# uiuc-iml/RA-SLAM

Hardware: AMD Instinct MI355X
Metric: depth+semantic frames/sec integrated @640x480, 5mm voxels (higher is better)
Workload: dtype f32

## Files before the change

ra-slam_amd/csrc/kernels_cand.h:

```cpp
#pragma once
#include "kernels_alloc.h"

namespace ratsdf {

constexpr int kCandSegs = 64;
constexpr int kCandCountStride = 32;
constexpr uint32_t kCandReserve = 32;
constexpr unsigned long long kCandEmpty = ~0ull;


struct CandJob {
  FrameParams P;
  const float* depth;
  const uint8_t* rgb;
  const float* ht;
  const float* lt;
  float4* texA;
  uint32_t* texB;
  CandSet set;
  uint32_t first_tile, n_tiles;
  uint32_t tiles_per_wg;
  uint32_t tiles_x;
  uint32_t tiles_x_magic;
};
inline uint32_t cand_tiles_magic(uint32_t tiles_x) { return tiles_x > 1 ? 0xFFFFFFFFu / tiles_x + 1u : 0u; }

constexpr uint32_t kCandLdsSlots = 512;

struct CandLds {
  unsigned long long keys[kCandLdsSlots];
  uint32_t ranks[kCandLdsSlots];
  uint32_t n, base;
};

__device__ inline void cand_append(const CandSet& cs, uint32_t seg, uint32_t k0, uint32_t k1,
                                   uint32_t rank, Ctl* ctl) {
  const uint32_t pos = atomicAdd(&cs.count[seg * kCandCountStride], 1u);
  if (pos < cs.seg_cap) {
    cs.list[(size_t)seg * cs.seg_cap + pos] = make_uint4(k0, k1, rank, 0u);
  } else {
    set_error(ctl, RATSDF_ERR_CAPACITY);
  }
}

__device__ inline bool cand_lds_insert(CandLds& L, unsigned long long key, uint32_t h, uint32_t rank) {
  uint32_t s = h & (kCandLdsSlots - 1);
  for (uint32_t guard = 0; guard < 32; ++guard) {
    unsigned long long k = L.keys[s];
    if (k == kCandEmpty) k = atomicCAS(&L.keys[s], kCandEmpty, key);
    if (k == kCandEmpty || k == key) {
      atomicMin(&L.ranks[s], rank);
      return true;
    }
    s = (s + 1) & (kCandLdsSlots - 1);
  }
  return false;
}

template <typename Overflow>
__device__ inline void cand_pixel_work(const CandJob& J, CandLds& L, uint32_t wg, Ctl* ctl, uint32_t reserved_at,
                                       Overflow overflow) {
  const FrameParams& P = J.P;
  const uint32_t wave = (uint32_t)__builtin_amdgcn_readfirstlane((int)(threadIdx.x >> 6));
  const int lane = threadIdx.x & 63;
  if (J.tiles_per_wg == 4 && (wg | 15u) < (J.n_tiles + 3) / 4) wg = (wg & ~15u) | ((wg & 7u) << 1) | ((wg >> 3) & 1u);
  const uint32_t rel = wg * J.tiles_per_wg + wave;
  const uint32_t tile = J.first_tile + rel;
  const uint32_t sup = tile >> 2, sub = tile & 3u;
  const uint32_t srow = J.tiles_x > 1 ? __umulhi(sup, J.tiles_x_magic) : sup;
  const uint32_t scol = sup - srow * J.tiles_x;
  const int px = (int)scol * 16 + (lane & 15);
  const int py = (int)srow * 16 + (int)sub * 4 + (lane >> 4);
  const bool inb = wave < J.tiles_per_wg && rel < J.n_tiles && px < P.W && py < P.H;
  const int pix = inb ? py * P.W + px : 0;
  float d = 0.f, hv = 1.f, lv = 1.f;
  uint32_t c0 = 0, c1 = 0, c2 = 0;
#ifdef RATSDF_STAMPS
  unsigned long long pt[5];
  pt[0] = clock64();
#endif
  if (inb) {
    c0 = J.rgb[3 * pix];
    c1 = J.rgb[3 * pix + 1];
    c2 = J.rgb[3 * pix + 2];
    d = J.depth[pix];
    if (P.has_sem) {
      hv = J.ht[pix];
      lv = J.lt[pix];
    }
  }
  const uint32_t c = c0 | (c1 << 8) | (c2 << 16);

  if (threadIdx.x == 0) L.base = reserved_at;
  const V3 pimg{(float)px, (float)py, 1.f};
  const V3 pc = intr_mul(P.Ki, pimg);
  const float r = sqrtf(pc.x * pc.x + (pc.y * pc.y + pc.z * pc.z));
  if (inb) {
    float ln = 0.f;
    if (P.has_sem) ln = __logf(hv) - __logf(lv);
    const Recip rmd = make_recip(P.md);
    const float wn = (1 - (recip_safe(P.md) ? div_shared(d, rmd) : d / P.md)) * 4;
    J.texA[pix] = make_float4(d, r, ln, wn);
    J.texB[pix] = c;
  }
  bool valid = inb && !(d == 0 || d > P.md);
  if (RATSDF_DBG(P, 1)) return;
#ifdef RATSDF_STAMPS
  pt[1] = clock64();
#endif

  const V3 pcd{pc.x * d, pc.y * d, pc.z * d};
  const V3 pw = se3_apply(P.Ti, pcd);
  if (P.shard_count > 1) {
    const float lo = (pw.x - P.trunc) / P.vs - 2.5f, hi = (pw.x + P.trunc) / P.vs + 2.5f;
    if (lo > -32000.f && hi < 32000.f) {
      const int s_lo = ((int)floorf(lo) >> 3) >> P.shard_slab_bits, s_hi = ((int)floorf(hi) >> 3) >> P.shard_slab_bits;
      const uint32_t u = (uint32_t)(s_lo + P.shard_bias);
      const uint32_t m_lo = u - __umulhi(u, P.shard_magic) * (uint32_t)P.shard_count;
      uint32_t k0 = (uint32_t)P.shard_rank + (uint32_t)P.shard_count - m_lo;
      if (k0 >= (uint32_t)P.shard_count) k0 -= (uint32_t)P.shard_count;
      if (k0 > (uint32_t)(s_hi - s_lo)) valid = false;
    }
    if (!__any(valid)) return;
  }
  const Recip rr = make_recip(r), rvs = make_recip(P.vs);
  const bool vs_ok = recip_safe(P.vs);
  const V3 dc{div_shared(pc.x, rr), div_shared(pc.y, rr), div_shared(pc.z, rr)};
  const V3 dw = quat_rotate(P.Ti.q, dc);
  const V3 sw{pw.x - dw.x * P.trunc, pw.y - dw.y * P.trunc, pw.z - dw.z * P.trunc};
  V3 dg, sg;
  if (vs_ok && __all(fabsf(sw.x) < 1e18f && fabsf(sw.y) < 1e18f && fabsf(sw.z) < 1e18f)) {
    dg = V3{div_shared(dw.x, rvs), div_shared(dw.y, rvs), div_shared(dw.z, rvs)};
    sg = V3{div_shared(sw.x, rvs), div_shared(sw.y, rvs), div_shared(sw.z, rvs)};
  } else {
    dg = V3{dw.x / P.vs, dw.y / P.vs, dw.z / P.vs};
    sg = V3{sw.x / P.vs, sw.y / P.vs, sw.z / P.vs};
  }
  const float two_tr = 2 * P.trunc;
  const V3 rg{two_tr * dg.x, two_tr * dg.y, two_tr * dg.z};
  int steps = f2i(ceilf(fmaxf(fmaxf(fabsf(rg.x), fabsf(rg.y)), fabsf(rg.z)) / RATSDF_BLOCK_LEN));
// ... 34 lines not shown
    const uint32_t k0 = act ? key0(bx, by) : kInf;
    const uint32_t k1 = act ? key1(bz) : kInf;
    const uint32_t n0 = (uint32_t)__builtin_amdgcn_update_dpp(0, (int)k0, 0x138, 0xF, 0xF, false);
    const uint32_t n1 = (uint32_t)__builtin_amdgcn_update_dpp(0, (int)k1, 0x138, 0xF, 0xF, false);
    const bool dup = (k0 == prev0 && k1 == prev1) || (lane > 0 && k0 == n0 && k1 == n1);
    if (act && !dup && shard_owned(bx, P) && !RATSDF_DBG(P, 2)) {
      const uint32_t rank = (uint32_t)pix * (uint32_t)P.S + (uint32_t)i;
      const unsigned long long key = (unsigned long long)k0 | ((unsigned long long)k1 << 32);
      if (!cand_lds_insert(L, key, (uint32_t)(bx + by * 17 + bz * 41), rank)) overflow(bx, by, bz, k0, k1, rank);
    }
    if (act) {
      prev0 = k0;
      prev1 = k1;
    }
    p.x += st.x;
    p.y += st.y;
    p.z += st.z;
#ifdef RATSDF_STAMPS
    pt[4] += 1;
#endif
  }
#ifdef RATSDF_STAMPS
  pt[3] = clock64();
  if (threadIdx.x == 0 && (wg & 15) == 0) {
    atomicAdd(&ctl->tstamps[11], pt[1] - pt[0]);
    atomicAdd(&ctl->tstamps[12], pt[2] - pt[1]);
    atomicAdd(&ctl->tstamps[13], pt[3] - pt[2]);
    atomicAdd(&ctl->tstamps[14], pt[4]);
    atomicAdd(&ctl->tstamps[15], 1ull);
  }
#endif
}

__device__ inline void cand_pixels_role(const CandJob& J, uint32_t wg, Ctl* ctl, CandLds& L) {
  const uint32_t nthreads = block_threads();
  for (uint32_t i = threadIdx.x; i < kCandLdsSlots; i += nthreads) {
    L.keys[i] = kCandEmpty;
    L.ranks[i] = kInf;
  }
  const uint32_t seg = (J.first_tile + wg) & (kCandSegs - 1);
  const uint32_t reserve = kCandReserve * ((J.tiles_per_wg + 3) / 4);
  uint32_t reserved_at = 0;
  if (threadIdx.x == 0) {
    L.n = 0;
    uint32_t opaque_zero;
    asm("v_mov_b32 %0, 0" : "=v"(opaque_zero));
    reserved_at = atomicAdd(&J.set.count[seg * kCandCountStride + opaque_zero], reserve);
  }
#ifdef RATSDF_STAMPS
  unsigned long long cs[4];
  cs[0] = clock64();
  unsigned long long* ws = (ctl->debug_buf && RATSDF_DBG(J.P, 8))
                               ? ctl->debug_buf + (size_t)(((J.first_tile / 4 + wg) * 4 + (threadIdx.x >> 6)) & 16383) * 8
                               : nullptr;
  if (ws && (threadIdx.x & 63) == 0) { ws[0] = cs[0]; ws[5] = wall_clock64(); }
#endif
  asm volatile("s_waitcnt lgkmcnt(0)\n\ts_barrier" ::: "memory");
#ifdef RATSDF_STAMPS
  cs[1] = clock64();
#endif
  if ((threadIdx.x >> 6) < J.tiles_per_wg)
    cand_pixel_work(J, L, wg, ctl, reserved_at, [&](int, int, int, uint32_t k0, uint32_t k1, uint32_t rank) {
      cand_append(J.set, (J.first_tile + wg) & (kCandSegs - 1), k0, k1, rank, ctl);
    });
#ifdef RATSDF_STAMPS
  cs[2] = clock64();
#endif
  asm volatile("s_waitcnt lgkmcnt(0)\n\ts_barrier" ::: "memory");
#ifdef RATSDF_STAMPS
  cs[3] = clock64();
  if (threadIdx.x == 0 && (wg & 15) == 0) {
    atomicAdd(&ctl->stamps[14], cs[1] - cs[0]);
    atomicAdd(&ctl->stamps[15], cs[2] - cs[1]);
    atomicAdd(&ctl->stamps[16], cs[3] - cs[2]);
    atomicAdd(&ctl->stamps[17], 1ull);
  }
#endif
  constexpr uint32_t kMaxPerThread = kCandLdsSlots / 64;
  uint32_t pos[kMaxPerThread];
#pragma unroll
  for (uint32_t k = 0; k < kMaxPerThread; ++k) {
    pos[k] = kInf;
    if (k * nthreads < kCandLdsSlots) {
      const uint32_t i = threadIdx.x + k * nthreads;
      if (i < kCandLdsSlots && L.keys[i] != kCandEmpty) pos[k] = atomicAdd(&L.n, 1u);
    }
  }
  asm volatile("s_waitcnt lgkmcnt(0)\n\ts_barrier" ::: "memory");
  const uint32_t n = L.n;
  const uint32_t base = L.base;
  uint32_t base2 = 0;
  if (n > reserve) {
    __syncthreads();
    if (threadIdx.x == 0) L.base = atomicAdd(&J.set.count[seg * kCandCountStride], n - reserve);
    __syncthreads();
    base2 = L.base;
  }
  if (base + reserve > J.set.seg_cap || (n > reserve && base2 + (n - reserve) > J.set.seg_cap)) {
    if (threadIdx.x == 0) set_error(ctl, RATSDF_ERR_CAPACITY);
    return;
  }
  uint4* out = J.set.list + (size_t)seg * J.set.seg_cap;
#pragma unroll
  for (uint32_t k = 0; k < kMaxPerThread; ++k) {
    const uint32_t i = threadIdx.x + k * nthreads;
    if (pos[k] != kInf) {
      const unsigned long long key = L.keys[i];
      const uint32_t at = pos[k] < reserve ? base + pos[k] : base2 + (pos[k] - reserve);
      out[at] = make_uint4((uint32_t)key, (uint32_t)(key >> 32), L.ranks[i], 0u);
    }
  }
  for (uint32_t i = n + threadIdx.x; i < reserve; i += nthreads)
    out[base + i] = make_uint4(kInf, kInf, kInf, 0u);
#ifdef RATSDF_STAMPS
  if (threadIdx.x == 0 && (wg & 15) == 0) atomicAdd(&ctl->stamps[18], (unsigned long long)clock64() - cs[3]);
  if (ws && (threadIdx.x & 63) == 0) {
    ws[1] = cs[1]; ws[2] = cs[2]; ws[3] = cs[3]; ws[4] = clock64(); ws[6] = wall_clock64();
  }
#endif
}

__device__ inline bool wave_block_visible_full(bool want, int bx, int by, int bz,
                                               const FrameParams& P) {
  const int lane = threadIdx.x & 63;
  unsigned long long todo = __ballot(want);
  unsigned long long ok = 0;
  while (todo) {
    unsigned long long packed = 0;
#pragma unroll
    for (int k = 0; k < 8; ++k) {
      unsigned long long o = 0xFFull;
      if (todo) {
        o = (unsigned long long)(__ffsll((long long)todo) - 1);
        todo &= todo - 1;
      }
      packed |= o << (8 * k);
    }
    const uint32_t own = (uint32_t)(packed >> (8 * (lane >> 3))) & 0xFFu;
    const int src = own == 0xFFu ? 0 : (int)own;
    const int cbx = __shfl(bx, src), cby = __shfl(by, src), cbz = __shfl(bz, src);
    const int c = lane & 7;
    const int cx = (int16_t)((int16_t)(cbx << 3) + ((c >> 0) & 1) * 7);
    const int cy = (int16_t)((int16_t)(cby << 3) + ((c >> 1) & 1) * 7);
    const int cz = (int16_t)((int16_t)(cbz << 3) + ((c >> 2) & 1) * 7);
    const bool v = own == 0xFFu || voxel_visible(cx, cy, cz, P);
    const unsigned long long b = __ballot(v);
#pragma unroll
    for (int k = 0; k < 8; ++k) {
      const unsigned long long o = (packed >> (8 * k)) & 0xFFull;
      if (o != 0xFFull && ((b >> (8 * k)) & 0xFFull) == 0xFFull) ok |= 1ull << o;
    }
  }
// ... 97 lines not shown
```

ra-slam_amd/csrc/kernels_frame.h:

```cpp
#pragma once
#include "kernels_integrate.h"

namespace ratsdf {

struct FrameJob {
  FrameParams P;
  const float* depth;
  const uint8_t* rgb;
  const float* ht;
  const float* lt;
  uint32_t par;
  uint32_t pad;
};
typedef const FrameJob __attribute__((address_space(4))) * JobPtr;

struct AheadGeom {
  uint32_t first_tile, n_tiles, tiles_per_wg, tiles_x, tiles_x_magic;
};

__device__ inline CandJob make_cand_job(EnginePtr E, JobPtr J, const AheadGeom& g) {
  CandJob j;
  j.P = ld_const(&J->P);
  j.depth = J->depth;
  j.rgb = J->rgb;
  j.ht = J->ht;
  j.lt = J->lt;
  const uint32_t par = J->par;
  j.texA = E->texA[par];
  j.texB = E->texB[par];
  j.set = ld_const(&E->cand[par]);
  j.first_tile = g.first_tile;
  j.n_tiles = g.n_tiles;
  j.tiles_per_wg = g.tiles_per_wg;
  j.tiles_x = g.tiles_x;
  j.tiles_x_magic = g.tiles_x_magic;
  return j;
}

constexpr uint32_t kFrontLdsWords = 2 * kSmallCarve + 16;
constexpr uint32_t kTailPerThread = 8;
constexpr uint32_t kTailReqMax = kTailPerThread * 256;
constexpr uint32_t kTailWinMax = kFreshCap;
constexpr uint32_t kTailBins = 512;
constexpr uint32_t kTailLdsWords = 32 + 5 * kTailWinMax;
static_assert(kTailBins <= kTailWinMax && kTailBins == 2 * 256, "two bins per thread; the cursors' memory is reused");

__device__ inline bool front_arrive(FrameCtl* F, uint32_t wg, uint32_t n_wg, Ctl* ctl) {
  __shared__ uint32_t arrived_last;
#ifdef RATSDF_STAMPS
  __shared__ unsigned long long arrive_t[3];
  if (threadIdx.x == 0) arrive_t[0] = wall_clock64();
#endif
  asm volatile("s_waitcnt vmcnt(0)" ::: "memory");
  __syncthreads();
#ifdef RATSDF_STAMPS
  if (threadIdx.x == 0) arrive_t[1] = wall_clock64();
#endif
  if (threadIdx.x == 0) {
    const uint32_t sub = wg % kArriveSubs;
    const uint32_t members = (n_wg - sub + kArriveSubs - 1) / kArriveSubs;
    uint32_t last = 0;
    if (__hip_atomic_fetch_add(&F->arrive[sub * kListStride], 1u, __ATOMIC_RELAXED, __HIP_MEMORY_SCOPE_AGENT) ==
        members - 1u) {
      const uint32_t tops = n_wg < kArriveSubs ? n_wg : kArriveSubs;
      last = __hip_atomic_fetch_add(&F->arrive_top, 1u, __ATOMIC_RELAXED, __HIP_MEMORY_SCOPE_AGENT) == tops - 1u;
    }
    arrived_last = last;
#ifdef RATSDF_STAMPS
// ... 212 lines not shown
    F->alloc_base = (uint32_t)nf;
    F->n_win = take;
    F->n_winlist = total;
    F->pending = 1;
    F->front_done = 1;
    ctl->num_free = nf - (int32_t)take;
    atomicMin(&ctl->free_low, nf - (int32_t)take);
    atomicAdd(&ctl->paths[0], 1ull);
#ifdef RATSDF_STAMPS
    tt[3] = wall_clock64();
    const unsigned long long T0 = __hip_atomic_load(&ctl->tstamps[0], __ATOMIC_RELAXED, __HIP_MEMORY_SCOPE_AGENT);
    for (int i = 0; i < 4; ++i) ctl->tstamps[4 + i] += tt[i] - T0;
    ctl->tstamps[8] += 1;
    ctl->tstamps[9] += n;
    ctl->tstamps[10] += total;
#endif
  }
}

template <bool kTail, typename Ahead>
__device__ inline void front_body(const Table& tab, const FrameParams& P, uint32_t n_vis_wg,
                                  const CandSet& cand, uint32_t cand_parts, Request* req,
                                  uint32_t req_cap, SlowRequest* slow, uint32_t slow_cap, VisItem* vis,
                                  uint32_t seg_cap, const Pool& pool, const CarveBufs& cb, Ctl* ctl,
                                  uint32_t par, ratsdf_frame_stats* stats, uint32_t tail, Ahead ahead,
                                  uint32_t* role_lds) {
  static_assert(sizeof(CandLds) <= kFrontLdsWords * 4 && kVisListCap <= 2 * kSmallCarve &&
                    sizeof(ReqBuf) <= kFrontLdsWords * 4,
                "role LDS");
  const uint32_t n_cons_wg = kCandSegs * cand_parts;
  const uint32_t n_dir_wg = n_vis_wg + n_cons_wg + kReleaseWGs;
  if (blockIdx.x >= n_dir_wg) {
    const CandJob job = ahead();
    cand_pixels_role(job, blockIdx.x - n_dir_wg, ctl, *reinterpret_cast<CandLds*>(role_lds));
    return;
  }
  FrameCtl* F = &ctl->fr[par];
  FrameCtl* Fp = &ctl->fr[par ^ 1u];
  if (kTail && (tail & 2u)) __builtin_amdgcn_s_setprio(3);
#ifdef RATSDF_STAMPS
  if (blockIdx.x == 0 && threadIdx.x == 0)
    __hip_atomic_store(&ctl->tstamps[0], (unsigned long long)wall_clock64(), __ATOMIC_RELAXED, __HIP_MEMORY_SCOPE_AGENT);
#endif
  bool expired = false;
  auto gate = [&]() {
    const GateResult g = carve_resolve_gate(tab, cb, ctl, Fp, RATSDF_DBG(P, 20));
    expired = expired || g == kGateExpired;
    return g;
  };
  if (blockIdx.x >= n_vis_wg + n_cons_wg) {
    if (!RATSDF_DBG(P, 12) && gate() != kGateExpired)
      carve_release_role(tab, pool, cb, ctl, Fp, blockIdx.x - n_vis_wg - n_cons_wg, role_lds);
  } else if (blockIdx.x >= n_vis_wg) {
    if (!RATSDF_DBG(P, 11)) {
      const uint32_t c = blockIdx.x - n_vis_wg;
      cand_consume_role(tab, P, cand, c % kCandSegs, c / kCandSegs, cand_parts, req, req_cap, slow,
                        slow_cap, ctl, F, gate, *reinterpret_cast<ReqBuf*>(role_lds));
    }
  } else {
    if (!RATSDF_DBG(P, 3)) visible_append_role(tab, P, blockIdx.x, n_vis_wg, vis, seg_cap, ctl, F, gate, role_lds);
  }
  if constexpr (kTail) {
    if ((tail & 1u) && !expired && front_arrive(F, blockIdx.x, n_dir_wg, ctl))
      front_tail_role(tab, P, cand, req, req_cap, vis, seg_cap, pool, cb, ctl, par, stats, role_lds);
  }
}

template <bool kTail>
__global__ __launch_bounds__(256) __attribute__((amdgpu_num_sgpr(80), amdgpu_waves_per_eu(8))) void k_front(
    Table tab, FrameParams P, uint32_t n_vis_wg, CandSet cand, uint32_t cand_parts, Request* req,
    uint32_t req_cap,
    SlowRequest* slow, uint32_t slow_cap, VisItem* vis, uint32_t seg_cap, Pool pool, CarveBufs cb,
    Ctl* ctl, uint32_t par, ratsdf_frame_stats* stats, uint32_t tail, CandJob ahead) {
  __shared__ __attribute__((aligned(16))) uint32_t role_lds[kFrontLdsWords];
  front_body<kTail>(tab, P, n_vis_wg, cand, cand_parts, req, req_cap, slow, slow_cap, vis, seg_cap, pool, cb,
                    ctl, par, stats, tail, [&]() { return ahead; }, role_lds);
}

__global__ __launch_bounds__(256) __attribute__((amdgpu_num_sgpr(80), amdgpu_waves_per_eu(8))) void k_front_inline(
    Table tab, uint32_t n_vis_wg, uint32_t n_now_wg, Request* req, uint32_t req_cap, SlowRequest* slow,
    uint32_t slow_cap, VisItem* vis, uint32_t seg_cap, Pool pool, CarveBufs cb, Ctl* ctl, uint32_t par, CandJob now,
    CandJob ahead) {
  static_assert((kInlineReqOffsetWords * 4u + sizeof(ReqBuf)) <= kFrontLdsWords * 4u, "role LDS");
  __shared__ __attribute__((aligned(16))) uint32_t role_lds[kFrontLdsWords];
  const uint32_t n_dir_wg = n_vis_wg + n_now_wg + kReleaseWGs;
  if (blockIdx.x >= n_dir_wg) {
    cand_pixels_role(ahead, blockIdx.x - n_dir_wg, ctl, *reinterpret_cast<CandLds*>(role_lds));
    return;
  }
  FrameCtl* F = &ctl->fr[par];
  FrameCtl* Fp = &ctl->fr[par ^ 1u];
  auto gate = [&]() { return carve_resolve_gate(tab, cb, ctl, Fp, RATSDF_DBG(now.P, 20)); };
  if (blockIdx.x >= n_vis_wg + n_now_wg) {
    if (gate() != kGateExpired)
      carve_release_role(tab, pool, cb, ctl, Fp, blockIdx.x - n_vis_wg - n_now_wg, role_lds);
  } else if (blockIdx.x >= n_vis_wg) {
    cand_inline_role(now, blockIdx.x - n_vis_wg, tab, req, req_cap, slow, slow_cap, ctl, F, gate, role_lds);
  } else {
    visible_append_role(tab, now.P, blockIdx.x, n_vis_wg, vis, seg_cap, ctl, F, gate, role_lds);
  }
}

template <bool kTail>
__global__ __launch_bounds__(256) __attribute__((amdgpu_num_sgpr(80), amdgpu_waves_per_eu(8))) void k_front_g(
    EnginePtr engs, JobPtr cur, JobPtr nxt, uint32_t n_vis_wg, uint32_t cand_parts, uint32_t tail, AheadGeom ag) {
  __shared__ __attribute__((aligned(16))) uint32_t role_lds[kFrontLdsWords];
  EnginePtr E = engs + blockIdx.y;
  JobPtr J = cur + blockIdx.y;
  const uint32_t par = J->par;
  const RankBufs rb = ld_const(&E->rb);
  front_body<kTail>(ld_const(&E->tab), ld_const(&J->P), n_vis_wg, ld_const(&E->cand[par]), cand_parts, rb.req,
             rb.req_cap, E->slow, E->slow_cap, E->vis, E->seg_cap, ld_const(&E->pool),
             ld_const(&E->cb[par ^ 1u]), E->ctl, par, E->stats, tail,
             [&]() { return make_cand_job(E, nxt + blockIdx.y, ag); }, role_lds);
}

__device__ inline void serial_frame_role(const Table& tab, const Pool& pool, const RankBufs& rb,
                                         const CarveBufs& cb, Ctl* ctl, uint32_t par,
                                         ratsdf_frame_stats* stats, unsigned long long* skeys) {
#ifdef RATSDF_STAMPS
// ... 162 lines not shown
  cand_pixels_role(job, blockIdx.x, E->ctl, L);
}

template <int VPL, bool kTail>
__global__ __launch_bounds__(VPL == 1 ? 512 : RATSDF_INTEG_NT) __attribute__((amdgpu_num_sgpr(80), amdgpu_waves_per_eu(VPL <= 2 ? 8 : (VPL == 4 ? 5 : 3)))) void k_integrate_g(
    EnginePtr engs, JobPtr cur, JobPtr nxt, uint32_t n_int_wg, uint32_t n_serial_wg, uint32_t n_ahead_wg,
    uint32_t commit_rot, AheadGeom ag) {
  constexpr bool tail_on = kTail;
  __shared__ __attribute__((aligned(16))) uint32_t role_lds[kIntegLdsWords];
  EnginePtr E = engs + blockIdx.y;
  JobPtr J = cur + blockIdx.y;
  const uint32_t par = J->par;
  if (__builtin_expect(blockIdx.x >= n_serial_wg + n_ahead_wg, 1)) {
    const uint32_t ibid = blockIdx.x - n_serial_wg - n_ahead_wg;
    const bool fused = n_serial_wg != 0;
    IntegArgs A;
    A.rgbw = E->pool.rgbw;
    A.tsdf = E->pool.tsdf;
    A.segm = E->pool.segm;
    A.texA = E->texA[par];
    A.texB = E->texB[par];
    A.vis = E->vis;
    A.seg_cap = E->seg_cap;
    A.F = &E->ctl->fr[par];
    A.upd_wg = E->cb[par].upd_wg;
    A.par = par;
    const FrameParams P = ld_const(&J->P);
#include "integrate_body.inc"
    return;
  }
  if (blockIdx.x >= n_serial_wg) {
    if (VPL != 1) {
      const CandJob ahead = make_cand_job(E, nxt + blockIdx.y, ag);
      cand_pixels_role(ahead, blockIdx.x - n_serial_wg, E->ctl, *reinterpret_cast<CandLds*>(role_lds));
    }
    return;
  }
  if (blockIdx.x == 0) {
    const uint32_t nwords = ((uint32_t)(J->P.W * J->P.H) * (uint32_t)J->P.S + 31u) / 32u;
    serial_workgroup(E, par, nwords, role_lds, RATSDF_DBG(J->P, 21));
  } else {
    serial_helper(E, par, role_lds, blockIdx.x, RATSDF_DBG(J->P, 22));
  }
}

}
```

ra-slam_amd/csrc/kernels_integrate.h:

```cpp
#pragma once
#include "kernels_carve.h"

namespace ratsdf {

template <typename Op>
__device__ inline uint32_t wave_reduce_dpp(uint32_t v, uint32_t identity, Op op) {
  v = op(v, (uint32_t)__builtin_amdgcn_update_dpp((int)identity, (int)v, 0xB1, 0xF, 0xF, false));
  v = op(v, (uint32_t)__builtin_amdgcn_update_dpp((int)identity, (int)v, 0x4E, 0xF, 0xF, false));
  v = op(v, (uint32_t)__builtin_amdgcn_update_dpp((int)identity, (int)v, 0x141, 0xF, 0xF, false));
  v = op(v, (uint32_t)__builtin_amdgcn_update_dpp((int)identity, (int)v, 0x140, 0xF, 0xF, false));
  v = op(v, (uint32_t)__builtin_amdgcn_update_dpp((int)identity, (int)v, 0x142, 0xA, 0xF, false));
  v = op(v, (uint32_t)__builtin_amdgcn_update_dpp((int)identity, (int)v, 0x143, 0xC, 0xF, false));
  return (uint32_t)__builtin_amdgcn_readlane((int)v, 63);
}
__device__ inline uint32_t wave_sum(uint32_t v) {
  return wave_reduce_dpp(v, 0u, [](uint32_t a, uint32_t b) { return a + b; });
}

template <int N>
struct VecIO;
template <>
struct VecIO<8> {
  static __device__ inline void load(const uint32_t* p, uint32_t (&v)[8]) {
    const uint4 a = reinterpret_cast<const uint4*>(p)[0], b = reinterpret_cast<const uint4*>(p)[1];
// ... 688 lines not shown
  }
}

#ifndef RATSDF_INTEG_NT
#define RATSDF_INTEG_NT 256
#endif

struct IntegArgs {
  uint32_t* rgbw;
  float* tsdf;
  float* segm;
  const float4* texA;
  const uint32_t* texB;
  const VisItem* vis;
  uint32_t seg_cap;
  FrameCtl* F;
  uint32_t* upd_wg;
  uint32_t par;
};

template <int VPL, bool kTail>
__global__ __launch_bounds__(VPL == 1 ? 512 : RATSDF_INTEG_NT) __attribute__((amdgpu_num_sgpr(80), amdgpu_waves_per_eu(VPL <= 2 ? 8 : (VPL == 4 ? 5 : 3)))) void k_integrate(
    IntegArgs A, FrameParams P, EnginePtr E, uint32_t n_int_wg, uint32_t n_serial_wg, uint32_t n_ahead_wg,
    uint32_t commit_rot, CandJob ahead) {
  constexpr bool tail_on = kTail;
  __shared__ __attribute__((aligned(16))) uint32_t role_lds[kIntegLdsWords];
  if (__builtin_expect(blockIdx.x >= n_serial_wg + n_ahead_wg, 1)) {
    const uint32_t ibid = blockIdx.x - n_serial_wg - n_ahead_wg;
    const bool fused = n_serial_wg != 0;
#include "integrate_body.inc"
    return;
  }
  if (blockIdx.x >= n_serial_wg) {
    if (VPL != 1) cand_pixels_role(ahead, blockIdx.x - n_serial_wg, E->ctl, *reinterpret_cast<CandLds*>(role_lds));
    return;
  }
  if (blockIdx.x == 0)
    serial_workgroup(E, A.par, ((uint32_t)(P.W * P.H) * (uint32_t)P.S + 31u) / 32u, role_lds, RATSDF_DBG(P, 21));
  else
    serial_helper(E, A.par, role_lds, blockIdx.x, RATSDF_DBG(P, 22));
}

}
```

ra-slam_amd/csrc/ratsdf_engine.hip:

```cpp
#include <hip/hip_runtime.h>
#include <hip/hip_ext.h>

#include <cmath>
#include <cstdio>
#include <cstdlib>
#include <cstring>
#include <new>
#include <algorithm>
#include <atomic>
#include <condition_variable>
#include <mutex>
#include <thread>
#include <vector>

#include "kernels_frame.h"
#include "kernels_mesh.h"
#include "kernels_sample.h"
#include "kernels_esdf.h"
#include "kernels_fuse.h"
#include "hip_mem.h"
#include "../../include/ratsdf_sample.h"
#include "../../include/ratsdf_esdf.h"

static_assert(sizeof(ratsdf_sample) == 32 && offsetof(ratsdf_sample, flags) == 25, "ratsdf_sample layout");
// ... 384 lines not shown
  int ensure_stage(size_t npix);
  EngineDev record() const;
  int upload_record();
  RankBufs rank_bufs(uint32_t nranks) const;
  int alloc_rank(uint32_t nranks, unsigned par, const CandJob* next = nullptr, bool frame = false);
  int commit_pass(uint32_t nranks, unsigned par);
  int settle();
  void abandon_pipeline(int frames_launched = 0, bool clear_next = false);
  CarveBufs carve_bufs(unsigned par) const;
  int select(int mode, const GridBounds& gb, uint32_t* count_slot);
  struct FrameIn {
    const void *rgb, *depth, *ht, *lt;
    const ratsdf_intrinsics* K;
    const ratsdf_pose* T;
    static FrameIn of(const void* rgb, const void* depth, const void* ht, const void* lt, const ratsdf_intrinsics* K,
                      const ratsdf_pose* T) {
      if (!ht || !lt) ht = lt = nullptr;
      return FrameIn{rgb, depth, ht, lt, K, T};
    }
    static FrameIn at(size_t i, const void* const* rgb, const void* const* depth, const void* const* ht,
                      const void* const* lt, const ratsdf_intrinsics* K, const ratsdf_pose* T) {
      return of(rgb[i], depth[i], ht ? ht[i] : nullptr, lt ? lt[i] : nullptr, &K[i], &T[i]);
    }
  };
  FrameParams frame_params(const FrameIn& in, int H, int W, float md) const;
  void fill_job(FrameJob& j, const FrameIn& in, int H, int W, float md, unsigned par) const;
  CandJob cand_job(const FrameIn& in, const FrameParams& P, unsigned par) const;
  int frame(const FrameIn& cur, const FrameIn* next, int H, int W, float md);
  int sticky();
  int read_small(void* dst, const void* dev_src, size_t bytes);
  FrameParams base_params() const;
  struct Geom {
    unsigned n_vis_wg, parts, n_front_wg, n_cand_wg, grid;
    AheadGeom a, b, c;
  };
  Geom geometry(int H, int W, bool has_next, int split_a, int split_b) const;
  int lookahead_split(size_t npix) const;
  bool graph_eligible(int n, int H, int W) const;
  struct StageSlot {
    uint8_t *h, *d;
    size_t npix;
    FrameIn input(const ratsdf_intrinsics* K, const ratsdf_pose* T, bool sem) const {
      return FrameIn{d + npix * 12, d, sem ? d + npix * 4 : nullptr, sem ? d + npix * 8 : nullptr, K, T};
    }
  };
  StageSlot stage_slot(int slot, size_t npix) const;
  void stage_fill(const StageSlot& s, const void* rgb, const void* depth, const void* ht, const void* lt, int parts);
  int stage_upload(const StageSlot& s, bool sem, hipStream_t cs);
  int stage_fail(int status);
};

FrameParams ratsdf_engine::base_params() const {
  FrameParams P;
  memset(&P, 0, sizeof(P));
  P.T = Se3{Quat{0, 0, 0, 1}, V3{0, 0, 0}};
  P.Ti = P.T;
  P.K = Intr{1, 1, 0, 0};
  P.Ki = P.K;
  P.vs = vs;
  P.trunc = trunc;
  P.md = 0;
  P.W = P.H = 0;
  P.S = 1;
  P.has_sem = 0;
  P.segm_live = 1;
  P.shard_rank = shard_rank;
// ... 282 lines not shown
  P.S = S;
  P.has_sem = (in.ht && in.lt) ? 1 : 0;
  if (P.has_sem) ever_sem = true;
  P.segm_live = ever_sem ? 1 : 0;
  return P;
}

void ratsdf_engine::fill_job(FrameJob& j, const FrameIn& in, int H, int W, float md, unsigned par) const {
  j.P = frame_params(in, H, W, md);
  j.depth = (const float*)in.depth;
  j.rgb = (const uint8_t*)in.rgb;
  j.ht = (const float*)in.ht;
  j.lt = (const float*)in.lt;
  j.par = par & 1u;
  j.pad = 0;
}

CandJob ratsdf_engine::cand_job(const FrameIn& in, const FrameParams& P, unsigned par) const {
  CandJob j;
  memset(&j, 0, sizeof(j));
  j.P = P;
  j.depth = (const float*)in.depth;
  j.rgb = (const uint8_t*)in.rgb;
  j.ht = (const float*)in.ht;
  j.lt = (const float*)in.lt;
  j.texA = texA[par];
  j.texB = texB[par];
  j.set = cand[par];
  j.tiles_x = (uint32_t)((P.W + 15) / 16);
  j.tiles_x_magic = cand_tiles_magic(j.tiles_x);
  j.first_tile = 0;
  j.n_tiles = j.tiles_x * (uint32_t)((P.H + 15) / 16) * 4u;
  j.tiles_per_wg = 4;
  return j;
}

ratsdf_engine::Geom ratsdf_engine::geometry(int H, int W, bool has_next, int split_a,
                                            int split_b) const {
  Geom g;
  memset(&g, 0, sizeof(g));
  const size_t npix = (size_t)H * W;
  const uint32_t tiles_x = (uint32_t)((W + 15) / 16);
  const uint32_t tiles = tiles_x * (uint32_t)((H + 15) / 16) * 4u;
  g.n_cand_wg = (tiles + 3) / 4;
  g.a.tiles_x = g.b.tiles_x = g.c.tiles_x = tiles_x;
  g.a.tiles_x_magic = g.b.tiles_x_magic = g.c.tiles_x_magic = cand_tiles_magic(tiles_x);
  g.a.tiles_per_wg = g.b.tiles_per_wg = g.c.tiles_per_wg = 4;
  if (has_next) {
    const uint32_t tiles_a = (uint32_t)((uint64_t)(tiles / 4) * (unsigned)split_a / 100) / 16 * 64;
    uint32_t tiles_b = (uint32_t)((uint64_t)(tiles / 4) * (unsigned)split_b / 100) / 16 * 64;
    if (split_a + split_b >= 100 || tiles_a + tiles_b > tiles) tiles_b = tiles - tiles_a;
    g.a.n_tiles = tiles_a;
    g.b.first_tile = tiles_a;
    g.b.n_tiles = tiles_b;
    const uint32_t tpw = (tiles_b + cand_wgs - 1) / cand_wgs;
    g.b.tiles_per_wg = std::min<uint32_t>(std::max<uint32_t>(tpw, 1u), 16u);
    g.c.first_tile = tiles_a + tiles_b;
    g.c.n_tiles = tiles - tiles_a - tiles_b;
  }
  g.n_vis_wg = std::min<unsigned>(128u, std::max<unsigned>(1u, ((unsigned)tab.num_block + 2 * 256 - 1) / (2 * 256)));
  const unsigned supers = ((unsigned)W + 15) / 16 * (((unsigned)H + 15) / 16);
  unsigned parts = (supers * kCandReserve / kCandSegs + 255) / 256;
  if (vs < 0.004f) parts *= 2;
  parts = std::min(std::max(parts, 1u), 32u);
  if (cand_parts_env) parts = cand_parts_env;
  g.parts = parts;
  g.n_front_wg = g.n_vis_wg + kCandSegs * parts + kReleaseWGs + (g.a.n_tiles + 3) / 4;
  g.grid = grid_from_env ? integrate_grid : (npix >= 600000 ? (unsigned)RATSDF_GRID_HD : (unsigned)RATSDF_GRID_VGA);
  return g;
}

int ratsdf_engine::lookahead_split(size_t npix) const {
  if (vpl == 1) return 100;
  return (int)(!cand_split_env && npix >= 600000 ? (unsigned)RATSDF_CAND_SPLIT_HD : cand_split);
}

bool ratsdf_engine::graph_eligible(int n, int H, int W) const {
  return use_graphs && n >= 2 && !cand_ready && fused_serial && vpl != 1 && (size_t)H * W * (size_t)S < 0xFFFFFFFFull;
}

int ratsdf_engine::frame(const FrameIn& cur, const FrameIn* next, int H, int W, float md) {
  const size_t npix = (size_t)H * W;
  if (npix * (size_t)S >= 0xFFFFFFFFull) return RATSDF_ERR_BAD_ARGUMENT;
  int st = ensure_image(npix, npix * (size_t)S);
  if (st != RATSDF_OK) return st;
  const FrameParams P = frame_params(cur, H, W, md);
  const unsigned par = parity;

  const bool inline_cand = !cand_ready;
#ifdef RATSDF_STAMPS
  const bool inline_kernel = inline_cand && !tab.tail_on && !inline_off;
  if (inline_cand && !inline_kernel) {
    const CandJob job = cand_job(cur, P, par);
    hipLaunchKernelGGL(k_cand, dim3((job.n_tiles + 3) / 4), dim3(256), 0, stream, job, ctl);
  }
#else
  const bool inline_kernel = inline_cand;
#endif
  const int split_b = (fused_serial && vpl != 1) ? 0 : (int)(cand_split_env ? cand_split_b : 0u);
  const Geom g = geometry(H, W, next != nullptr, lookahead_split(npix), split_b);
  CandJob ahead_a, ahead_b, ahead_c;
  memset(&ahead_a, 0, sizeof(ahead_a));
  memset(&ahead_b, 0, sizeof(ahead_b));
  memset(&ahead_c, 0, sizeof(ahead_c));
  if (next) {
    const FrameParams Pn = frame_params(*next, H, W, md);
    ahead_a = cand_job(*next, Pn, par ^ 1u);
    ahead_b = ahead_a;
    ahead_c = ahead_a;
    auto set = [](CandJob& j, const AheadGeom& ag) {
      j.first_tile = ag.first_tile;
      j.n_tiles = ag.n_tiles;
      j.tiles_per_wg = ag.tiles_per_wg;
    };
    set(ahead_a, g.a);
    set(ahead_b, g.b);
    set(ahead_c, g.c);
  }
  parity = par ^ 1u;
  cand_ready = next != nullptr;

  const bool fused = fused_serial && vpl != 1;
  if (inline_kernel) {
    const CandJob now = cand_job(cur, P, par);
    const unsigned n_now_wg = (now.n_tiles + 3) / 4;
    hipLaunchKernelGGL(k_front_inline, dim3(g.n_vis_wg + n_now_wg + kReleaseWGs + (g.a.n_tiles + 3) / 4), dim3(256), 0,
                       stream, tab, (uint32_t)g.n_vis_wg, (uint32_t)n_now_wg, req, req_cap, slow, kSlowCap,
                       vis + kFreshCap, seg_cap, pool, carve_bufs(par ^ 1u), ctl, (uint32_t)par, now, ahead_a);
  } else
#ifdef RATSDF_STAMPS
  if (tab.tail_on)
    hipLaunchKernelGGL(k_front<true>, dim3(g.n_front_wg), dim3(256), 0, stream, tab, P, g.n_vis_wg, cand[par],
                       (uint32_t)g.parts, req, req_cap, slow, kSlowCap, vis + kFreshCap, seg_cap, pool,
                       carve_bufs(par ^ 1u), ctl, (uint32_t)par, d_stats, 1u | front_prio, ahead_a);
  else
#endif
    hipLaunchKernelGGL(k_front<false>, dim3(g.n_front_wg), dim3(256), 0, stream, tab, P, g.n_vis_wg, cand[par],
                       (uint32_t)g.parts, req, req_cap, slow, kSlowCap, vis + kFreshCap, seg_cap, pool,
                       carve_bufs(par ^ 1u), ctl, (uint32_t)par, d_stats, 0u, ahead_a);
#ifdef RATSDF_STAMPS
  if (sort_lists) {
    HIPCHK(hipStreamSynchronize(stream));
    std::vector<uint32_t> fc(sizeof(FrameCtl) / 4);
    HIPCHK(hipMemcpy(fc.data(), &ctl->fr[par], sizeof(FrameCtl), hipMemcpyDeviceToHost));
    const FrameCtl* hf = reinterpret_cast<const FrameCtl*>(fc.data());
    const double qx = P.T.q.x, qy = P.T.q.y, qz = P.T.q.z, qw = P.T.q.w;
    for (int l = 0; l < kNumLists; ++l) {
      uint32_t n = hf->n_list[l * kListStride];
      if (n > seg_cap - kFreshCap) n = seg_cap - kFreshCap;
      if (n < 2) continue;
      std::vector<VisItem> items(n);
      VisItem* dl = vis + kFreshCap + (size_t)l * seg_cap;
      HIPCHK(hipMemcpy(items.data(), dl, (size_t)n * sizeof(VisItem), hipMemcpyDeviceToHost));
      auto key = [&](const VisItem& it) {
        const double x = (it.x * 8 + 4) * (double)P.vs, y = (it.y * 8 + 4) * (double)P.vs, z = (it.z * 8 + 4) * (double)P.vs;
        const double ux = 2 * (qy * z - qz * y), uy = 2 * (qz * x - qx * z), uz = 2 * (qx * y - qy * x);
        const double cx = x + qw * ux + (qy * uz - qz * uy) + P.T.t.x, cy = y + qw * uy + (qz * ux - qx * uz) + P.T.t.y,
                     cz = z + qw * uz + (qx * uy - qy * ux) + P.T.t.z;
        double u = (P.K.fx * cx + P.K.cx * cz) / cz, v = (P.K.fy * cy + P.K.cy * cz) / cz;
// ... 780 lines not shown
```

Measured before the change: 39400.

## Split lookahead candidate work into texel prep in front kernel and ray stage in integrate

The candidate-generation work for the next frame is split into two phases. Texel preparation (loading depth/rgb/semantics, computing ray norm and weights, writing texA/texB) for the integrate-share tiles now runs in extra front-kernel workgroups. The integrate kernel's share then only reads depth and ray norm back from texA and does the ray marching. The goal is to take global loads and log math off the integrate kernel's critical path. The cost is extra front workgroups and a texA round trip through memory.

```diff
diff --git a/ra-slam_amd/csrc/kernels_cand.h b/ra-slam_amd/csrc/kernels_cand.h
--- a/ra-slam_amd/csrc/kernels_cand.h
+++ b/ra-slam_amd/csrc/kernels_cand.h
@@ -22,6 +22,7 @@
   uint32_t tiles_per_wg;
   uint32_t tiles_x;
   uint32_t tiles_x_magic;
+  uint32_t tex_first, tex_tiles;
 };
 inline uint32_t cand_tiles_magic(uint32_t tiles_x) { return tiles_x > 1 ? 0xFFFFFFFFu / tiles_x + 1u : 0u; }
 
@@ -57,55 +58,82 @@
   return false;
 }
 
-template <typename Overflow>
-__device__ inline void cand_pixel_work(const CandJob& J, CandLds& L, uint32_t wg, Ctl* ctl, uint32_t reserved_at,
-                                       Overflow overflow) {
+struct CandPix {
+  int px, py, pix;
+  bool inb;
+};
+__device__ inline CandPix cand_tile_pixel(const CandJob& J, uint32_t first_tile, uint32_t n_tiles, uint32_t wg) {
   const FrameParams& P = J.P;
   const uint32_t wave = (uint32_t)__builtin_amdgcn_readfirstlane((int)(threadIdx.x >> 6));
   const int lane = threadIdx.x & 63;
-  if (J.tiles_per_wg == 4 && (wg | 15u) < (J.n_tiles + 3) / 4) wg = (wg & ~15u) | ((wg & 7u) << 1) | ((wg >> 3) & 1u);
+  if (J.tiles_per_wg == 4 && (wg | 15u) < (n_tiles + 3) / 4) wg = (wg & ~15u) | ((wg & 7u) << 1) | ((wg >> 3) & 1u);
   const uint32_t rel = wg * J.tiles_per_wg + wave;
-  const uint32_t tile = J.first_tile + rel;
+  const uint32_t tile = first_tile + rel;
   const uint32_t sup = tile >> 2, sub = tile & 3u;
   const uint32_t srow = J.tiles_x > 1 ? __umulhi(sup, J.tiles_x_magic) : sup;
   const uint32_t scol = sup - srow * J.tiles_x;
-  const int px = (int)scol * 16 + (lane & 15);
-  const int py = (int)srow * 16 + (int)sub * 4 + (lane >> 4);
-  const bool inb = wave < J.tiles_per_wg && rel < J.n_tiles && px < P.W && py < P.H;
-  const int pix = inb ? py * P.W + px : 0;
+  CandPix q;
+  q.px = (int)scol * 16 + (lane & 15);
+  q.py = (int)srow * 16 + (int)sub * 4 + (lane >> 4);
+  q.inb = wave < J.tiles_per_wg && rel < n_tiles && q.px < P.W && q.py < P.H;
+  q.pix = q.inb ? q.py * P.W + q.px : 0;
+  return q;
+}
+
+struct CandInputs {
+  float d, hv, lv;
+  uint32_t c;
+};
+__device__ inline CandInputs cand_texel_load(const CandJob& J, const CandPix& q) {
+  const FrameParams& P = J.P;
   float d = 0.f, hv = 1.f, lv = 1.f;
   uint32_t c0 = 0, c1 = 0, c2 = 0;
+  if (q.inb) {
+    c0 = J.rgb[3 * q.pix];
+    c1 = J.rgb[3 * q.pix + 1];
+    c2 = J.rgb[3 * q.pix + 2];
+    d = J.depth[q.pix];
+    if (P.has_sem) {
+      hv = J.ht[q.pix];
+      lv = J.lt[q.pix];
+    }
+  }
+  return CandInputs{d, hv, lv, c0 | (c1 << 8) | (c2 << 16)};
+}
+__device__ inline V3 cand_pixel_ray(const FrameParams& P, const CandPix& q) {
+  return intr_mul(P.Ki, V3{(float)q.px, (float)q.py, 1.f});
+}
+__device__ inline float cand_ray_norm(const V3& pc) { return sqrtf(pc.x * pc.x + (pc.y * pc.y + pc.z * pc.z)); }
+__device__ inline void cand_texel_store(const CandJob& J, const CandPix& q, const CandInputs& in, float r) {
+  const FrameParams& P = J.P;
+  if (q.inb) {
+    float ln = 0.f;
+    if (P.has_sem) ln = __logf(in.hv) - __logf(in.lv);
+    const Recip rmd = make_recip(P.md);
+    const float wn = (1 - (recip_safe(P.md) ? div_shared(in.d, rmd) : in.d / P.md)) * 4;
+    J.texA[q.pix] = make_float4(in.d, r, ln, wn);
+    J.texB[q.pix] = in.c;
+  }
+}
+
+__device__ inline void cand_texel_role(const CandJob& J, uint32_t wg) {
+  const CandPix q = cand_tile_pixel(J, J.tex_first, J.tex_tiles, wg);
+  const CandInputs in = cand_texel_load(J, q);
+  cand_texel_store(J, q, in, cand_ray_norm(cand_pixel_ray(J.P, q)));
+}
+
+template <typename Overflow>
+__device__ inline void cand_ray_work(const CandJob& J, CandLds& L, const CandPix& q, float d, float r, const V3& pc,
+                                     [[maybe_unused]] uint32_t wg, Ctl* ctl, Overflow overflow,
+                                     [[maybe_unused]] unsigned long long t0) {
+  const FrameParams& P = J.P;
+  const int lane = threadIdx.x & 63;
+  const int pix = q.pix;
+  bool valid = q.inb && !(d == 0 || d > P.md);
+  if (RATSDF_DBG(P, 1)) return;
 #ifdef RATSDF_STAMPS
   unsigned long long pt[5];
-  pt[0] = clock64();
-#endif
-  if (inb) {
-    c0 = J.rgb[3 * pix];
-    c1 = J.rgb[3 * pix + 1];
-    c2 = J.rgb[3 * pix + 2];
-    d = J.depth[pix];
-    if (P.has_sem) {
-      hv = J.ht[pix];
-      lv = J.lt[pix];
-    }
-  }
-  const uint32_t c = c0 | (c1 << 8) | (c2 << 16);
-
-  if (threadIdx.x == 0) L.base = reserved_at;
-  const V3 pimg{(float)px, (float)py, 1.f};
-  const V3 pc = intr_mul(P.Ki, pimg);
-  const float r = sqrtf(pc.x * pc.x + (pc.y * pc.y + pc.z * pc.z));
-  if (inb) {
-    float ln = 0.f;
-    if (P.has_sem) ln = __logf(hv) - __logf(lv);
-    const Recip rmd = make_recip(P.md);
-    const float wn = (1 - (recip_safe(P.md) ? div_shared(d, rmd) : d / P.md)) * 4;
-    J.texA[pix] = make_float4(d, r, ln, wn);
-    J.texB[pix] = c;
-  }
-  bool valid = inb && !(d == 0 || d > P.md);
-  if (RATSDF_DBG(P, 1)) return;
-#ifdef RATSDF_STAMPS
+  pt[0] = t0;
   pt[1] = clock64();
 #endif
 
@@ -206,6 +234,40 @@
 #endif
 }
 
+template <typename Overflow>
+__device__ inline void cand_pixel_work(const CandJob& J, CandLds& L, uint32_t wg, Ctl* ctl, uint32_t reserved_at,
+                                       Overflow overflow) {
+  const CandPix q = cand_tile_pixel(J, J.first_tile, J.n_tiles, wg);
+#ifdef RATSDF_STAMPS
+  const unsigned long long t0 = clock64();
+#else
+  const unsigned long long t0 = 0;
+#endif
+  const CandInputs in = cand_texel_load(J, q);
+  if (threadIdx.x == 0) L.base = reserved_at;
+  const V3 pc = cand_pixel_ray(J.P, q);
+  const float r = cand_ray_norm(pc);
+  cand_texel_store(J, q, in, r);
+  cand_ray_work(J, L, q, in.d, r, pc, wg, ctl, overflow, t0);
+}
+
+template <typename Overflow>
+__device__ inline void cand_ray_work_staged(const CandJob& J, CandLds& L, uint32_t wg, Ctl* ctl, uint32_t reserved_at,
+                                            Overflow overflow) {
+  const CandPix q = cand_tile_pixel(J, J.first_tile, J.n_tiles, wg);
+#ifdef RATSDF_STAMPS
+  const unsigned long long t0 = clock64();
+#else
+  const unsigned long long t0 = 0;
+#endif
+  float2 dr = make_float2(0.f, 1.f);
+  if (q.inb) dr = *reinterpret_cast<const float2*>(J.texA + q.pix);
+  if (threadIdx.x == 0) L.base = reserved_at;
+  const V3 pc = cand_pixel_ray(J.P, q);
+  cand_ray_work(J, L, q, dr.x, dr.y, pc, wg, ctl, overflow, t0);
+}
+
+template <bool kStaged = false>
 __device__ inline void cand_pixels_role(const CandJob& J, uint32_t wg, Ctl* ctl, CandLds& L) {
   const uint32_t nthreads = block_threads();
   for (uint32_t i = threadIdx.x; i < kCandLdsSlots; i += nthreads) {
@@ -233,10 +295,13 @@
 #ifdef RATSDF_STAMPS
   cs[1] = clock64();
 #endif
-  if ((threadIdx.x >> 6) < J.tiles_per_wg)
-    cand_pixel_work(J, L, wg, ctl, reserved_at, [&](int, int, int, uint32_t k0, uint32_t k1, uint32_t rank) {
+  if ((threadIdx.x >> 6) < J.tiles_per_wg) {
+    auto overflow = [&](int, int, int, uint32_t k0, uint32_t k1, uint32_t rank) {
       cand_append(J.set, (J.first_tile + wg) & (kCandSegs - 1), k0, k1, rank, ctl);
-    });
+    };
+    if constexpr (kStaged) cand_ray_work_staged(J, L, wg, ctl, reserved_at, overflow);
+    else cand_pixel_work(J, L, wg, ctl, reserved_at, overflow);
+  }
 #ifdef RATSDF_STAMPS
   cs[2] = clock64();
 #endif
@@ -292,6 +357,19 @@
     ws[1] = cs[1]; ws[2] = cs[2]; ws[3] = cs[3]; ws[4] = clock64(); ws[6] = wall_clock64();
   }
 #endif
+}
+
+__device__ inline void cand_rays_role(const CandJob& J, uint32_t wg, Ctl* ctl, CandLds& L) {
+  cand_pixels_role<true>(J, wg, ctl, L);
+}
+
+#ifndef RATSDF_PHASE_SPLIT
+#define RATSDF_PHASE_SPLIT 1
+#endif
+constexpr bool kPhaseSplit = RATSDF_PHASE_SPLIT != 0;
+__device__ inline void cand_integrate_share(const CandJob& J, uint32_t wg, Ctl* ctl, CandLds& L) {
+  if constexpr (kPhaseSplit) cand_rays_role(J, wg, ctl, L);
+  else cand_pixels_role(J, wg, ctl, L);
 }
 
 __device__ inline bool wave_block_visible_full(bool want, int bx, int by, int bz,
diff --git a/ra-slam_amd/csrc/kernels_frame.h b/ra-slam_amd/csrc/kernels_frame.h
--- a/ra-slam_amd/csrc/kernels_frame.h
+++ b/ra-slam_amd/csrc/kernels_frame.h
@@ -15,8 +15,14 @@
 typedef const FrameJob __attribute__((address_space(4))) * JobPtr;
 
 struct AheadGeom {
-  uint32_t first_tile, n_tiles, tiles_per_wg, tiles_x, tiles_x_magic;
+  uint32_t first_tile, n_tiles, tiles_per_wg, tiles_x, tiles_x_magic, tex_first, tex_tiles;
 };
+
+__device__ inline void front_ahead_role(const CandJob& job, uint32_t wg, Ctl* ctl, uint32_t* role_lds) {
+  const uint32_t n_whole = (job.n_tiles + 3) / 4;
+  if (wg < n_whole) cand_pixels_role(job, wg, ctl, *reinterpret_cast<CandLds*>(role_lds));
+  else cand_texel_role(job, wg - n_whole);
+}
 
 __device__ inline CandJob make_cand_job(EnginePtr E, JobPtr J, const AheadGeom& g) {
   CandJob j;
@@ -34,6 +40,8 @@
   j.tiles_per_wg = g.tiles_per_wg;
   j.tiles_x = g.tiles_x;
   j.tiles_x_magic = g.tiles_x_magic;
+  j.tex_first = g.tex_first;
+  j.tex_tiles = g.tex_tiles;
   return j;
 }
 
@@ -312,7 +320,7 @@
   const uint32_t n_dir_wg = n_vis_wg + n_cons_wg + kReleaseWGs;
   if (blockIdx.x >= n_dir_wg) {
     const CandJob job = ahead();
-    cand_pixels_role(job, blockIdx.x - n_dir_wg, ctl, *reinterpret_cast<CandLds*>(role_lds));
+    front_ahead_role(job, blockIdx.x - n_dir_wg, ctl, role_lds);
     return;
   }
   FrameCtl* F = &ctl->fr[par];
@@ -365,7 +373,7 @@
   __shared__ __attribute__((aligned(16))) uint32_t role_lds[kFrontLdsWords];
   const uint32_t n_dir_wg = n_vis_wg + n_now_wg + kReleaseWGs;
   if (blockIdx.x >= n_dir_wg) {
-    cand_pixels_role(ahead, blockIdx.x - n_dir_wg, ctl, *reinterpret_cast<CandLds*>(role_lds));
+    front_ahead_role(ahead, blockIdx.x - n_dir_wg, ctl, role_lds);
     return;
   }
   FrameCtl* F = &ctl->fr[par];
@@ -594,7 +602,7 @@
   if (blockIdx.x >= n_serial_wg) {
     if (VPL != 1) {
       const CandJob ahead = make_cand_job(E, nxt + blockIdx.y, ag);
-      cand_pixels_role(ahead, blockIdx.x - n_serial_wg, E->ctl, *reinterpret_cast<CandLds*>(role_lds));
+      cand_integrate_share(ahead, blockIdx.x - n_serial_wg, E->ctl, *reinterpret_cast<CandLds*>(role_lds));
     }
     return;
   }
diff --git a/ra-slam_amd/csrc/kernels_integrate.h b/ra-slam_amd/csrc/kernels_integrate.h
--- a/ra-slam_amd/csrc/kernels_integrate.h
+++ b/ra-slam_amd/csrc/kernels_integrate.h
@@ -744,7 +744,7 @@
     return;
   }
   if (blockIdx.x >= n_serial_wg) {
-    if (VPL != 1) cand_pixels_role(ahead, blockIdx.x - n_serial_wg, E->ctl, *reinterpret_cast<CandLds*>(role_lds));
+    if (VPL != 1) cand_integrate_share(ahead, blockIdx.x - n_serial_wg, E->ctl, *reinterpret_cast<CandLds*>(role_lds));
     return;
   }
   if (blockIdx.x == 0)
diff --git a/ra-slam_amd/csrc/ratsdf_engine.hip b/ra-slam_amd/csrc/ratsdf_engine.hip
--- a/ra-slam_amd/csrc/ratsdf_engine.hip
+++ b/ra-slam_amd/csrc/ratsdf_engine.hip
@@ -440,6 +440,7 @@
   FrameParams base_params() const;
   struct Geom {
     unsigned n_vis_wg, parts, n_front_wg, n_cand_wg, grid;
+    unsigned n_ahead_front_wg;
     AheadGeom a, b, c;
   };
   Geom geometry(int H, int W, bool has_next, int split_a, int split_b) const;
@@ -788,6 +789,7 @@
   j.first_tile = 0;
   j.n_tiles = j.tiles_x * (uint32_t)((P.H + 15) / 16) * 4u;
   j.tiles_per_wg = 4;
+  j.tex_first = j.tex_tiles = 0;
   return j;
 }
 
@@ -803,7 +805,8 @@
   g.a.tiles_x_magic = g.b.tiles_x_magic = g.c.tiles_x_magic = cand_tiles_magic(tiles_x);
   g.a.tiles_per_wg = g.b.tiles_per_wg = g.c.tiles_per_wg = 4;
   if (has_next) {
-    const uint32_t tiles_a = (uint32_t)((uint64_t)(tiles / 4) * (unsigned)split_a / 100) / 16 * 64;
+    const uint32_t tiles_a =
+        split_a >= 100 ? tiles : (uint32_t)((uint64_t)(tiles / 4) * (unsigned)split_a / 100) / 16 * 64;
     uint32_t tiles_b = (uint32_t)((uint64_t)(tiles / 4) * (unsigned)split_b / 100) / 16 * 64;
     if (split_a + split_b >= 100 || tiles_a + tiles_b > tiles) tiles_b = tiles - tiles_a;
     g.a.n_tiles = tiles_a;
@@ -813,6 +816,10 @@
     g.b.tiles_per_wg = std::min<uint32_t>(std::max<uint32_t>(tpw, 1u), 16u);
     g.c.first_tile = tiles_a + tiles_b;
     g.c.n_tiles = tiles - tiles_a - tiles_b;
+    if (kPhaseSplit) {
+      g.a.tex_first = g.c.first_tile;
+      g.a.tex_tiles = g.c.n_tiles;
+    }
   }
   g.n_vis_wg = std::min<unsigned>(128u, std::max<unsigned>(1u, ((unsigned)tab.num_block + 2 * 256 - 1) / (2 * 256)));
   const unsigned supers = ((unsigned)W + 15) / 16 * (((unsigned)H + 15) / 16);
@@ -821,7 +828,8 @@
   parts = std::min(std::max(parts, 1u), 32u);
   if (cand_parts_env) parts = cand_parts_env;
   g.parts = parts;
-  g.n_front_wg = g.n_vis_wg + kCandSegs * parts + kReleaseWGs + (g.a.n_tiles + 3) / 4;
+  g.n_ahead_front_wg = (g.a.n_tiles + 3) / 4 + (g.a.tex_tiles + 3) / 4;
+  g.n_front_wg = g.n_vis_wg + kCandSegs * parts + kReleaseWGs + g.n_ahead_front_wg;
   g.grid = grid_from_env ? integrate_grid : (npix >= 600000 ? (unsigned)RATSDF_GRID_HD : (unsigned)RATSDF_GRID_VGA);
   return g;
 }
@@ -868,6 +876,8 @@
       j.first_tile = ag.first_tile;
       j.n_tiles = ag.n_tiles;
       j.tiles_per_wg = ag.tiles_per_wg;
+      j.tex_first = ag.tex_first;
+      j.tex_tiles = ag.tex_tiles;
     };
     set(ahead_a, g.a);
     set(ahead_b, g.b);
@@ -880,7 +890,7 @@
   if (inline_kernel) {
     const CandJob now = cand_job(cur, P, par);
     const unsigned n_now_wg = (now.n_tiles + 3) / 4;
-    hipLaunchKernelGGL(k_front_inline, dim3(g.n_vis_wg + n_now_wg + kReleaseWGs + (g.a.n_tiles + 3) / 4), dim3(256), 0,
+    hipLaunchKernelGGL(k_front_inline, dim3(g.n_vis_wg + n_now_wg + kReleaseWGs + g.n_ahead_front_wg), dim3(256), 0,
                        stream, tab, (uint32_t)g.n_vis_wg, (uint32_t)n_now_wg, req, req_cap, slow, kSlowCap,
                        vis + kFreshCap, seg_cap, pool, carve_bufs(par ^ 1u), ctl, (uint32_t)par, now, ahead_a);
   } else
```

Result: slower. 35780 (-9.2%).
